# EryiXie/PlaneRecNet

Hardware: AMD Instinct MI355X
Metric: img/s fwd+bwd @480×640 ResNet101-DCN, 1/2/4/8 MI355X + roofline % (higher is better)
Workload: dtype f32 (tensors and accumulation fp32; plain GEMMs and the tap-walked 4x4/s2, 1x1/s2 and sub-pixel convolutions >= 300 tiles: 2xfp16-piece split MFMA, fp32 accumulate; fp32-only rate in fp32_only_run)

## Files before the change

### include/prn.h

```cpp
#ifndef PRN_H
#define PRN_H
#include <stdint.h>
#ifdef __cplusplus
extern "C" {
#endif

#define PRN_BN_SPLITS 32

int prn_version(void);
const char* prn_last_error(void);

enum { PRN_IN_ZERO = 0, PRN_IN_REFLECT = 1, PRN_IN_UP2_REFLECT = 2, PRN_IN_DILATED = 3, PRN_IN_UP2_PHASE = 4,
       PRN_IN_EMBED1 = 5  };
enum { PRN_EPI_NONE = 0, PRN_EPI_RELU = 1, PRN_EPI_SIGMOID = 2 };

enum { PRN_SPLIT_OFF = 0, PRN_SPLIT_PLAN = 1, PRN_SPLIT_ALWAYS = 2 };
enum { PRN_PIECES_BF16 = 0, PRN_PIECES_F16 = 16 };
typedef struct prn_gemm_opts {
  int32_t split_mode;
  int32_t split_kind;
  int32_t split_products;
  int32_t split_min_tiles;
  float split_min_gflop;
  int32_t wgrad_wgs;
// ... 65 lines not shown
int prn_winograd_input(const float* x, float* V, int B, int C, int H, int W, int in_mode, void* stream);
int64_t prn_gemm_batched_ws_bytes(int M, int C, int P, int nb, const prn_gemm_opts* opts);
int prn_gemm_batched(int M, int C, int P, int nb, const float* U, const void* u_images, const float* V, float* Y, void* ws, const prn_gemm_opts* opts,
                     void* stream);
int prn_winograd_output(const float* Y, const float* bias, const float* addend, float* y, int B, int M, int H, int W, int epilogue, void* stream);
int prn_winograd_output_bn_fwd(const float* Yt, float* x_out, float* stats, const float* gamma, const float* beta, float* y, float* running_mean,
                               float* running_var, int B, int M, int H, int W, float eps, float momentum, int relu, void* stream);
int prn_winograd_output_bn_bwd(const float* Yt, const float* x, const float* stats, const float* gamma, const float* beta, float* dx, float* dgamma,
                               float* dbeta, int B, int M, int H, int W, int relu, void* stream);
int64_t prn_winograd_wgrad_ws_bytes(int B, int C, int H, int W, int M, const prn_gemm_opts* opts);
int prn_winograd_dy(const float* dy, float* Y, int B, int M, int H, int W, void* stream);
int prn_gemm_batched_nt_splits(int M, int C, int P, int nb, const prn_gemm_opts* opts);
int prn_gemm_batched_nt_kind(int M, int C, int P, int nb, const prn_gemm_opts* opts);
int prn_gemm_batched_nt(int M, int C, int P, int nb, const float* A, const float* Bm, float* ws, const prn_gemm_opts* opts, void* stream);
int prn_winograd_dw(const float* partials, float* dw, int M, int C, int splits, void* stream);
int prn_conv3x3_winograd_wgrad(const float* x, const float* dy, float* dw, void* ws, int B, int C, int H, int W, int M, int in_mode, const prn_gemm_opts* opts,
                               void* stream, int phase);
int prn_conv3x3_winograd_wgrad_v(const float* V, const float* dy, float* dw, void* ws, int B, int C, int H, int W, int M, const prn_gemm_opts* opts, void* stream);
int64_t prn_winograd_tiles_ragged(const prn_ragged* rg, int B);
int64_t prn_conv3x3_winograd_ragged_ws_bytes(const prn_ragged* rg, int B, int C, int M, const prn_gemm_opts* opts);
int prn_conv3x3_winograd_ragged(const float* x, const float* U, const void* u_images, const float* bias, const float* addend, float* y, void* ws,
                                const prn_ragged* rg, int B, int C, int M, int epilogue, const prn_gemm_opts* opts, void* stream);
int64_t prn_winograd_wgrad_ragged_ws_bytes(const prn_ragged* rg, int B, int C, int M, const prn_gemm_opts* opts);
int prn_conv3x3_winograd_wgrad_ragged(const float* x, const float* dy, float* dw, void* ws, const prn_ragged* rg, int B, int C, int M, const prn_gemm_opts* opts,
                                      void* stream);
int64_t prn_conv3x3_winograd_ws_bytes(int B, int C, int H, int W, int M, const prn_gemm_opts* opts);
int prn_conv3x3_winograd(const float* x, const float* U, const void* u_images, const float* bias, const float* addend, float* y, void* ws, int B, int C, int H,
                         int W, int M, int in_mode, int epilogue, const prn_gemm_opts* opts, void* stream);

int64_t prn_conv2d_wgrad_ws_bytes(const prn_conv_desc* d);
int prn_conv2d_wgrad_kernel_kind(const prn_conv_desc* d, int G);
int prn_conv2d_wgrad(const prn_conv_desc* d, const float* x, const float* dy, float* dw, void* ws, void* stream);
#define PRN_WGRAD_GROUP_MAX 16
int64_t prn_conv2d_wgrad_grouped_ws_bytes(const prn_conv_desc* d, int G);
int prn_conv2d_wgrad_grouped(const prn_conv_desc* d, int G, const float* const* x, const float* const* dy, float* dw, void* ws, void* stream);
int prn_conv2d_wgrad_phase(const prn_conv_desc* d, const float* x, const float* dy, float* dw, void* ws, void* stream, int phase);

int prn_up2_phase_weights(const float* w, float* wp, int M, int C, void* stream);
int prn_up2_dgrad_weights(const float* w, float* kd, int M, int C, void* stream);
int prn_replicate_fold(const float* dp, float* dx, int B, int C, int H, int W, void* stream);
int prn_space_to_depth2(const float* in, float* out, int B, int C, int H, int W, void* stream);
int prn_up2_wgrad_combine(const float* dwp, float* dw, int M, int C, void* stream);

int prn_pad_fold(const float* dp, float* dx, int B, int C, int H, int W, int up2, void* stream);
int prn_pad_fold_pitched(const float* dp, float* dx, int B, int C, int H, int W, int pitch, void* stream);

int prn_channel_sum(const float* x, float* out, double* ws, int B, int C, int HW, void* stream);

int prn_dcn_sample(const float* x, const float* om, float* cols, int B, int C, int H, int W, int Ho, int Wo,
                   int stride, float max_offset, void* stream);
int64_t prn_dcn_sample_bwd_ws_bytes(int B, int C, int H, int W, int Ho, int Wo);
int prn_dcn_sample_bwd(const float* x, const float* om, const float* dcols, float* dx, float* d_om, void* ws,
                       int B, int C, int H, int W, int Ho, int Wo, int stride, float max_offset, void* stream);

typedef struct prn_dcn_desc {
  int32_t B, C, H, W;
  int32_t M;
  int32_t stride, pad;
  int32_t Ho, Wo;
  int32_t raw;
  float max_offset;
  int32_t epilogue;
  prn_gemm_opts opts;
} prn_dcn_desc;
int64_t prn_dcnv2_table_bytes(const prn_dcn_desc* d);
int prn_dcnv2_table(const prn_dcn_desc* d, const float* offset, const float* mask, void* table, void* stream);
int64_t prn_dcnv2_fwd_ws_bytes(const prn_dcn_desc* d);
int prn_dcnv2_fwd(const prn_dcn_desc* d, const float* x, const void* table, const float* w, const float* bias, float* y, void* ws, void* stream);
int prn_dcnv2_fwd_phase(const prn_dcn_desc* d, const float* x, const void* table, const float* w, const float* bias, float* y, void* ws, void* stream,
                        int phase);
int64_t prn_dcnv2_bwd_weight_ws_bytes(const prn_dcn_desc* d);
int prn_dcnv2_bwd_weight(const prn_dcn_desc* d, const float* x, const void* table, const float* dy, float* dw, void* ws, void* stream);
int prn_dcnv2_bwd_weight_phase(const prn_dcn_desc* d, const float* x, const void* table, const float* dy, float* dw, void* ws, void* stream, int phase);
int64_t prn_dcnv2_bwd_ws_bytes(const prn_dcn_desc* d);
int prn_dcnv2_bwd_input(const prn_dcn_desc* d, const float* dy, const float* wt, const void* wt_images, const float* offset, const float* mask, float* dx,
                        void* ws, void* stream);
int prn_dcnv2_bwd_input_phase(const prn_dcn_desc* d, const float* dy, const float* wt, const void* wt_images, const float* offset, const float* mask,
                              float* dx, void* ws, void* stream, int phase);
int prn_dcnv2_bwd_offset_mask(const prn_dcn_desc* d, const float* x, const float* offset, const float* mask, float* d_offset, float* d_mask,
                              void* ws, void* stream);

int prn_bn_stats(const float* x, float* stats, float* running_mean, float* running_var, double* ws,
                 int B, int C, int HW, float eps, float momentum, void* stream);
int prn_bn_apply(const float* x, const float* stats, const float* gamma, const float* beta, const float* residual,
                 float* y, int B, int C, int HW, int relu, void* stream);
int prn_bn_kernel_kind(int B, int HW);
int prn_bn_train_fwd(const float* x, float* stats, const float* gamma, const float* beta, const float* residual, float* y,
                     float* running_mean, float* running_var, double* ws, int B, int C, int HW, float eps, float momentum,
                     int relu, void* stream);
int prn_bn_bwd(const float* dy, const float* x, const float* y, const float* stats, const float* gamma, const float* beta,
               float* dx, float* dres, float* dgamma, float* dbeta, double* ws,
               int B, int C, int HW, int relu, int frozen, void* stream);
int prn_bn_train_fwd_into(const float* x, float* stats, const float* gamma, const float* beta, const float* residual, float* y,
                          int64_t y_batch_stride, float* running_mean, float* running_var, double* ws, int B, int C, int HW, float eps,
                          float momentum, int relu, void* stream);
int prn_bn_bwd_from(const float* dy, int64_t dy_batch_stride, const float* x, const float* y, const float* stats, const float* gamma,
                    const float* beta, float* dx, float* dres, float* dgamma, float* dbeta, double* ws,
                    int B, int C, int HW, int relu, int frozen, void* stream);

int prn_bn_train_fwd_partials(const float* parts, int nparts, int64_t part_stride, float* x_out, float* stats, const float* gamma, const float* beta,
                              const float* residual, float* y, float* running_mean, float* running_var, int B, int C, int HW, float eps, float momentum,
                              int relu, void* stream);
int prn_bn_bwd_partials(const float* dparts, int nparts, int64_t part_stride, const float* x, const float* y, const float* stats, const float* gamma,
                        const float* beta, float* dx, float* dres, float* dgamma, float* dbeta, int B, int C, int HW, int relu, int frozen, void* stream);
int prn_bn_train_fwd_winograd(const float* parts, int nparts, int64_t part_stride, float* x_out, float* stats, const float* gamma, const float* beta,
                              const float* residual, float* y, float* running_mean, float* running_var, float* V, int B, int C, int H, int W, float eps,
// ... 196 lines not shown
```

### planerecnet_amd/_lib.py

```python
import ctypes
import os

_HERE = os.path.dirname(os.path.abspath(__file__))
LIB_PATH = os.environ.get("PRN_LIB") or os.path.join(_HERE, "libprn_hip.so")

c_int, c_float, c_void_p, c_i64 = ctypes.c_int, ctypes.c_float, ctypes.c_void_p, ctypes.c_int64


class GemmOpts(ctypes.Structure):
    _fields_ = [("split_mode", ctypes.c_int32), ("split_kind", ctypes.c_int32), ("split_products", ctypes.c_int32), ("split_min_tiles", ctypes.c_int32),
                ("split_min_gflop", ctypes.c_float), ("wgrad_wgs", ctypes.c_int32), ("wgrad_target", ctypes.c_int32), ("wgrad_split", ctypes.c_int32)]

    def key(self):
        return (self.split_mode, self.split_kind, self.split_products, self.split_min_tiles, self.split_min_gflop, self.wgrad_wgs, self.wgrad_target, self.wgrad_split)


SPLIT_OFF, SPLIT_PLAN, SPLIT_ALWAYS = 0, 1, 2
PIECES_BF16, PIECES_F16 = 0, 16


class ConvDesc(ctypes.Structure):
    _fields_ = [(n, ctypes.c_int32) for n in
                ("B", "C", "H", "W", "M", "KH", "KW", "stride", "pad", "Ho", "Wo", "in_mode", "dil", "epilogue", "ystride", "yH", "yW", "reserved")] + [
                    ("opts", GemmOpts)]
# ... 38 lines not shown
    "prn_split_images_bytes": (c_i64, [c_int, c_int, c_int]),
    "prn_split_prepare": (c_int, [P, P, c_int, c_int, c_int, c_int, P]),
    "prn_split_prepare_batched": (c_int, [P, c_int, c_i64, c_i64, c_int, P]),
    "prn_conv2d_fwd": (c_int, [_DP, P, P, P, P, P, P, P]),
    "prn_conv2d_fwd_ragged": (c_int, [_DP, P, P, P, P, P, P, P]),
    "prn_conv2d_wgrad_ragged_ws_bytes": (c_i64, [_DP, P]),
    "prn_conv2d_wgrad_ragged": (c_int, [_DP, P, P, P, P, P, P]),
    "prn_gn_relu_fwd_ragged": (c_int, [P, P, P, P, P, c_int, c_int, c_int, P, c_int, c_float, P]),
    "prn_gn_relu_bwd_ragged": (c_int, [P, P, P, P, P, P, P, P, c_int, c_int, c_int, P, c_int, P]),
    "prn_conv2d_fwd_phase": (c_int, [_DP, P, P, P, P, P, P, P, c_int]),
    "prn_conv2d_fwd_counted": (c_int, [_DP, P, P, P, P, P, P, P, P, P, c_int]),
    "prn_conv2d_wgrad_phase": (c_int, [_DP, P, P, P, P, P, c_int]),
    "prn_weight_flip_transpose": (c_int, [P, P, c_int, c_int, c_int, c_int, P]),
    "prn_weight_flip_transpose_batched": (c_int, [P, c_int, c_i64, P]),
    "prn_winograd_tiles": (c_i64, [c_int, c_int, c_int]),
    "prn_winograd_weights_batched": (c_int, [P, c_int, c_i64, P]),
    "prn_winograd_input": (c_int, [P, P, c_int, c_int, c_int, c_int, c_int, P]),
    "prn_gemm_batched_ws_bytes": (c_i64, [c_int, c_int, c_int, c_int, _OP]),
    "prn_gemm_batched": (c_int, [c_int, c_int, c_int, c_int, P, P, P, P, P, _OP, P]),
    "prn_winograd_output": (c_int, [P, P, P, P, c_int, c_int, c_int, c_int, c_int, P]),
    "prn_winograd_output_bn_fwd": (c_int, [P] * 8 + [c_int] * 4 + [c_float, c_float, c_int, P]),
    "prn_winograd_output_bn_bwd": (c_int, [P] * 8 + [c_int] * 5 + [P]),
    "prn_winograd_wgrad_ws_bytes": (c_i64, [c_int] * 5 + [_OP]),
    "prn_winograd_dy": (c_int, [P, P, c_int, c_int, c_int, c_int, P]),
    "prn_gemm_batched_nt_splits": (c_int, [c_int] * 4 + [_OP]),
    "prn_gemm_batched_nt_kind": (c_int, [c_int] * 4 + [_OP]),
    "prn_conv2d_wgrad_kernel_kind": (c_int, [_DP, c_int]),
    "prn_gemm_batched_nt": (c_int, [c_int, c_int, c_int, c_int, P, P, P, _OP, P]),
    "prn_winograd_dw": (c_int, [P, P, c_int, c_int, c_int, P]),
    "prn_conv3x3_winograd_wgrad": (c_int, [P, P, P, P, c_int, c_int, c_int, c_int, c_int, c_int, _OP, P, c_int]),
    "prn_winograd_tiles_ragged": (c_i64, [P, c_int]),
    "prn_conv3x3_winograd_ragged_ws_bytes": (c_i64, [P, c_int, c_int, c_int, _OP]),
    "prn_conv3x3_winograd_ragged": (c_int, [P, P, P, P, P, P, P, P, c_int, c_int, c_int, c_int, _OP, P]),
    "prn_winograd_wgrad_ragged_ws_bytes": (c_i64, [P, c_int, c_int, c_int, _OP]),
    "prn_conv3x3_winograd_wgrad_ragged": (c_int, [P, P, P, P, P, c_int, c_int, c_int, _OP, P]),
    "prn_conv3x3_winograd_wgrad_v": (c_int, [P, P, P, P, c_int, c_int, c_int, c_int, c_int, _OP, P]),
    "prn_conv3x3_winograd_ws_bytes": (c_i64, [c_int] * 5 + [_OP]),
    "prn_conv3x3_winograd": (c_int, [P, P, P, P, P, P, P, c_int, c_int, c_int, c_int, c_int, c_int, c_int, _OP, P]),
    "prn_conv2d_wgrad_ws_bytes": (c_i64, [_DP]),
    "prn_conv2d_wgrad_grouped_ws_bytes": (c_i64, [_DP, c_int]),
    "prn_conv2d_wgrad_grouped": (c_int, [_DP, c_int, P, P, P, P, P]),
    "prn_conv2d_wgrad": (c_int, [_DP, P, P, P, P, P]),
    "prn_pad_fold": (c_int, [P, P, c_int, c_int, c_int, c_int, c_int, P]),
    "prn_pad_fold_pitched": (c_int, [P, P, c_int, c_int, c_int, c_int, c_int, P]),
    "prn_up2_phase_weights": (c_int, [P, P, c_int, c_int, P]),
    "prn_up2_dgrad_weights": (c_int, [P, P, c_int, c_int, P]),
    "prn_up2_wgrad_combine": (c_int, [P, P, c_int, c_int, P]),
    "prn_space_to_depth2": (c_int, [P, P, c_int, c_int, c_int, c_int, P]),
    "prn_replicate_fold": (c_int, [P, P, c_int, c_int, c_int, c_int, P]),
    "prn_channel_sum": (c_int, [P, P, P, c_int, c_int, c_int, P]),
    "prn_dcn_sample": (c_int, [P, P, P] + [c_int] * 7 + [c_float, P]),
    "prn_dcn_sample_bwd_ws_bytes": (c_i64, [c_int] * 6),
    "prn_dcn_sample_bwd": (c_int, [P, P, P, P, P, P] + [c_int] * 7 + [c_float, P]),
    "prn_dcnv2_table_bytes": (c_i64, [P]),
    "prn_dcnv2_table": (c_int, [P, P, P, P, P]),
    "prn_dcnv2_fwd_ws_bytes": (c_i64, [P]),
    "prn_dcnv2_fwd": (c_int, [P] * 8),
    "prn_dcnv2_fwd_phase": (c_int, [P] * 8 + [c_int]),
    "prn_dcnv2_bwd_weight_ws_bytes": (c_i64, [P]),
    "prn_dcnv2_bwd_weight": (c_int, [P] * 7),
    "prn_dcnv2_bwd_weight_phase": (c_int, [P] * 7 + [c_int]),
    "prn_dcnv2_bwd_ws_bytes": (c_i64, [P]),
    "prn_dcnv2_bwd_input": (c_int, [P] * 9),
    "prn_dcnv2_bwd_input_phase": (c_int, [P] * 9 + [c_int]),
    "prn_bn_kernel_kind": (c_int, [c_int, c_int]),
    "prn_dcnv2_bwd_offset_mask": (c_int, [P] * 8),
    "prn_plane_prior_ws_bytes": (c_i64, [c_int] * 6 + [_OP]),
    "prn_plane_prior_fwd": (c_int, [P] * 7 + [c_int] * 6 + [_OP, P]),
    "prn_plane_prior_fwd_phase": (c_int, [P] * 7 + [c_int] * 6 + [_OP, P, c_int]),
    "prn_plane_prior_wgrad_ws_bytes": (c_i64, [c_int] * 5 + [_OP]),
    "prn_plane_prior_wgrad": (c_int, [P] * 4 + [c_int] * 5 + [_OP, P]),
    "prn_fpn_level_ws_bytes": (c_i64, [c_int] * 8 + [_OP]),
    "prn_fpn_level_fwd": (c_int, [P, P, P, P, c_int, c_int, P, P, P, P, P, P] + [c_int] * 6 + [_OP, P]),
    "prn_frame_to_input": (c_int, [P] + [c_int] * 6 + [P, P, c_int, P, P, P]),
    "prn_mask_loss_ws_floats": (c_int, [c_int]),
    "prn_mask_loss_fwd": (c_int, [P] * 9 + [c_int, c_int, c_int, c_float, c_float, P]),
    "prn_mask_loss_bwd": (c_int, [P] * 8 + [c_int, c_int, P]),
    "prn_vnl_triplets": (c_int, [P] * 12 + [c_int, c_int, c_int, c_float, P]),
    "prn_vnl_scatter": (c_int, [P] * 5 + [c_int, c_int, P]),
    "prn_depth_metrics_ws_doubles": (c_int, []),
    "prn_depth_metrics": (c_int, [P, P, P, P, c_i64, c_float, c_float, P]),
    "prn_vnl_trim_key": (c_int, [P, P, P, P, c_int, P]),
    "prn_vnl_trim_fwd": (c_int, [P, P, P, P, P, P, P, c_int, c_int, c_int, P, P, P, P, P, P]),
    "prn_vnl_trim_ws_bytes": (c_i64, [c_int]),
    "prn_vnl_trim_bwd": (c_int, [P, P, P, P, P, P, P, c_int, c_int, P, P]),
    "prn_loss_ws_doubles": (c_int, [c_int]),
    "prn_focal_sum_fwd": (c_int, [P, P, P, P, c_i64, c_int, c_float, c_float, P]),
    "prn_focal_sum_bwd": (c_int, [P, P, P, P, c_i64, c_int, c_float, c_float, P]),
    "prn_rmse_log_fwd": (c_int, [P, P, P, P, P, c_int, c_int, c_float, c_float, P]),
    "prn_rmse_log_bwd": (c_int, [P, P, P, P, P, c_int, c_int, c_float, c_float, P]),
    "prn_gt_segments": (c_i64, [c_int, c_int]),
    "prn_gt_mask_stats": (c_int, [P, P, c_int, c_int, c_int, c_int, P, P, P, P]),
    "prn_gt_quarter_masks": (c_int, [P, P, c_int, c_int, c_int, P]),
    "prn_gt_sample_triplets": (c_int, [P, P, c_int, c_int, c_int, c_int, P, P, P, P, P, ctypes.c_uint64, ctypes.c_uint64, c_i64, P, P]),
    "prn_adam_chunk_elems": (c_int, []),
    "prn_adam_step": (c_int, [P, c_int, c_int, P, P, P, P, P, P, P, P, P, ctypes.c_double, ctypes.c_double, c_float, P]),
    "prn_adam_step_masked": (c_int, [P, c_int, c_int, P, P, P, P, P, P, P, P, P, ctypes.c_double, ctypes.c_double, c_float, P, P, P]),
    "prn_pairwise_iou_ws_bytes": (c_i64, [c_int, c_int, c_i64]),
    "prn_pairwise_iou": (c_int, [P, P, P, P, c_int, c_int, c_i64, P, P, P, P]),
    "prn_mask_boxes": (c_int, [P, c_int, c_int, c_int, P, P]),
    "prn_mask_stats": (c_int, [P, c_int, c_i64, c_float, P, P, P]),
    "prn_sigmoid_point_nms": (c_int, [P, P, c_int, c_int, c_int, c_i64, P]),
    "prn_matrix_nms": (c_int, [P, P, P, c_int, c_float, c_int, P, P, P]),
    "prn_mask_nms_ws_bytes": (c_i64, [c_int, c_int, c_i64]),
    "prn_mask_nms": (c_int, [P, P, P, P, c_int, c_int, c_i64, c_float, P, P, P]),
    "prn_bn_stats": (c_int, [P, P, P, P, P, c_int, c_int, c_int, c_float, c_float, P]),
# ... 71 lines not shown
```

### planerecnet_amd/csrc/prn_dcn.hip

```cpp
#include <stdlib.h>
#include "prn_common.h"

namespace {

struct Tap {
  int i00, i01, i10, i11;
  float w00, w01, w10, w11;
  float gy00, gy01, gy10, gy11, gx00, gx01, gx10, gx11;
  float mod;
  float sig;
  bool pass_y, pass_x;
};

struct OmView {
  const float* off; const float* msk;
  int64_t off_bs, msk_bs;
  float maxoff;
  int raw, pad;
};

__device__ __forceinline__ Tap make_tap(const OmView& v, int b, int k, int ho, int wo, int Ho, int Wo,
                                        int H, int W, int stride, bool need_grad) {
  Tap t;
  const size_t plane = (size_t)Ho * Wo, pix = (size_t)ho * Wo + wo;
  const float* ob = v.off + (size_t)b * v.off_bs;
  const float ry = ob[(2 * k) * plane + pix], rx = ob[(2 * k + 1) * plane + pix];
  float dy = ry, dx = rx;
  t.pass_y = t.pass_x = true;
  if (v.raw) {
    const float maxoff = v.maxoff;
    const float rm = ob[(18 + k) * plane + pix];
    dy = fminf(fmaxf(ry, -maxoff), maxoff); dx = fminf(fmaxf(rx, -maxoff), maxoff);
    t.pass_y = (ry >= -maxoff) && (ry <= maxoff);
    t.pass_x = (rx >= -maxoff) && (rx <= maxoff);
    t.sig = 1.f / (1.f + expf(-rm));
    t.mod = 2.f * t.sig;
  } else {
    t.sig = 0.f;
    t.mod = v.msk ? v.msk[(size_t)b * v.msk_bs + (size_t)k * plane + pix] : 1.f;
  }
  const int ki = k / 3, kj = k - ki * 3;
  const float y = (float)(ho * stride - v.pad + ki) + dy, x = (float)(wo * stride - v.pad + kj) + dx;
  const bool inside = (y > -1.f) && (y < (float)H) && (x > -1.f) && (x < (float)W);
  const float fy = floorf(y), fx = floorf(x);
  const int y0 = (int)fy, x0 = (int)fx, y1 = y0 + 1, x1 = x0 + 1;
  const float ly = y - fy, lx = x - fx, hy = 1.f - ly, hx = 1.f - lx;
  const bool vy0 = inside && y0 >= 0, vy1 = inside && y1 <= H - 1, vx0 = x0 >= 0, vx1 = x1 <= W - 1;
  const bool v00 = vy0 && vx0, v01 = vy0 && vx1, v10 = vy1 && vx0, v11 = vy1 && vx1;
  t.i00 = v00 ? y0 * W + x0 : 0; t.i01 = v01 ? y0 * W + x1 : 0;
  t.i10 = v10 ? y1 * W + x0 : 0; t.i11 = v11 ? y1 * W + x1 : 0;
  t.w00 = v00 ? hy * hx : 0.f; t.w01 = v01 ? hy * lx : 0.f;
  t.w10 = v10 ? ly * hx : 0.f; t.w11 = v11 ? ly * lx : 0.f;
  if (need_grad) {
    t.gy00 = v00 ? -hx : 0.f; t.gy01 = v01 ? -lx : 0.f; t.gy10 = v10 ? hx : 0.f; t.gy11 = v11 ? lx : 0.f;
    t.gx00 = v00 ? -hy : 0.f; t.gx01 = v01 ? hy : 0.f; t.gx10 = v10 ? -ly : 0.f; t.gx11 = v11 ? ly : 0.f;
  }
  return t;
}

__global__ __launch_bounds__(256) void dcn_sample_kernel(const float* __restrict__ x, OmView om,
                                                         float* __restrict__ cols, int B, int C, int H, int W, int Ho,
                                                         int Wo, int stride) {
  const int64_t gid = (int64_t)blockIdx.x * blockDim.x + threadIdx.x;
  const int64_t plane = (int64_t)Ho * Wo;
  if (gid >= (int64_t)B * 9 * plane) return;
  const int pix = gid % plane, k = (gid / plane) % 9, b = gid / (9 * plane);
  const int ho = pix / Wo, wo = pix - ho * Wo;
  const Tap t = make_tap(om, b, k, ho, wo, Ho, Wo, H, W, stride, false);
  const int cper = (C + gridDim.y - 1) / gridDim.y;
  const int c0 = blockIdx.y * cper, c1 = min(C, c0 + cper);
  const size_t HW = (size_t)H * W;
  const float* xp = x + ((size_t)b * C + c0) * HW;
  float* cp = cols + (((size_t)b * C + c0) * 9 + k) * plane + pix;
  constexpr int UN = 8;
  int c = c0;
  for (; c + UN <= c1; c += UN) {
    float a00[UN], a01[UN], a10[UN], a11[UN];
#pragma unroll
    for (int u = 0; u < UN; ++u) {
      const float* q = xp + (size_t)u * HW;
      a00[u] = q[t.i00]; a01[u] = q[t.i01]; a10[u] = q[t.i10]; a11[u] = q[t.i11];
    }
    __builtin_amdgcn_sched_barrier(0);
#pragma unroll
    for (int u = 0; u < UN; ++u) cp[(size_t)u * 9 * plane] = t.mod * (t.w00 * a00[u] + t.w01 * a01[u] + t.w10 * a10[u] + t.w11 * a11[u]);
    xp += (size_t)UN * HW;
    cp += (size_t)UN * 9 * plane;
  }
  for (; c < c1; ++c) {
    const float v = t.w00 * xp[t.i00] + t.w01 * xp[t.i01] + t.w10 * xp[t.i10] + t.w11 * xp[t.i11];
    *cp = t.mod * v;
    xp += HW;
    cp += 9 * plane;
  }
}

__global__ __launch_bounds__(256) void dcn_dom_partial_kernel(const float* __restrict__ x, OmView om,
                                                              const float* __restrict__ dcols, float* __restrict__ part, int B,
                                                              int C, int H, int W, int Ho, int Wo, int stride) {
  const int64_t gid = (int64_t)blockIdx.x * blockDim.x + threadIdx.x;
  const int64_t plane = (int64_t)Ho * Wo;
  if (gid >= (int64_t)B * 9 * plane) return;
  const int pix = gid % plane, k = (gid / plane) % 9, b = gid / (9 * plane);
  const int ho = pix / Wo, wo = pix - ho * Wo;
  const Tap t = make_tap(om, b, k, ho, wo, Ho, Wo, H, W, stride, true);
  const int cper = (C + gridDim.y - 1) / gridDim.y;
  const int c0 = blockIdx.y * cper, c1 = min(C, c0 + cper);
  const size_t HW = (size_t)H * W;
  const float* xp = x + ((size_t)b * C + c0) * HW;
  const float* dp = dcols + (((size_t)b * C + c0) * 9 + k) * plane + pix;
  float gy = 0.f, gx = 0.f, gm = 0.f;
  constexpr int UN = 8;
  int c = c0;
  for (; c + UN <= c1; c += UN) {
    float g[UN], a00[UN], a01[UN], a10[UN], a11[UN];
#pragma unroll
    for (int u = 0; u < UN; ++u) {
      const float* q = xp + (size_t)u * HW;
      g[u] = dp[(size_t)u * 9 * plane];
      a00[u] = q[t.i00]; a01[u] = q[t.i01]; a10[u] = q[t.i10]; a11[u] = q[t.i11];
    }
    __builtin_amdgcn_sched_barrier(0);
#pragma unroll
    for (int u = 0; u < UN; ++u) {
      gm += g[u] * (t.w00 * a00[u] + t.w01 * a01[u] + t.w10 * a10[u] + t.w11 * a11[u]);
      gy += g[u] * (t.gy00 * a00[u] + t.gy01 * a01[u] + t.gy10 * a10[u] + t.gy11 * a11[u]);
      gx += g[u] * (t.gx00 * a00[u] + t.gx01 * a01[u] + t.gx10 * a10[u] + t.gx11 * a11[u]);
    }
    xp += (size_t)UN * HW;
    dp += (size_t)UN * 9 * plane;
  }
  for (; c < c1; ++c) {
    const float g = *dp;
    const float x00 = xp[t.i00], x01 = xp[t.i01], x10 = xp[t.i10], x11 = xp[t.i11];
    gm += g * (t.w00 * x00 + t.w01 * x01 + t.w10 * x10 + t.w11 * x11);
    gy += g * (t.gy00 * x00 + t.gy01 * x01 + t.gy10 * x10 + t.gy11 * x11);
    gx += g * (t.gx00 * x00 + t.gx01 * x01 + t.gx10 * x10 + t.gx11 * x11);
    xp += HW;
    dp += 9 * plane;
  }
  float* ob = part + ((size_t)blockIdx.y * B + b) * 27 * plane + pix;
  ob[(2 * k) * plane] = t.pass_y ? gy * t.mod : 0.f;
  ob[(2 * k + 1) * plane] = t.pass_x ? gx * t.mod : 0.f;
  ob[(18 + k) * plane] = om.raw ? gm * 2.f * t.sig * (1.f - t.sig) : gm;
}

__global__ void dcn_dom_final_kernel(const float* __restrict__ part, float* __restrict__ d_off, float* __restrict__ d_msk, int64_t n, int G,
                                     int plane) {
  const int64_t i = (int64_t)blockIdx.x * blockDim.x + threadIdx.x;
  if (i >= n) return;
  float s = 0.f;
  for (int g = 0; g < G; ++g) s += part[(size_t)g * n + i];
  if (d_msk == nullptr) { d_off[i] = s; return; }
  const int64_t b = i / (27 * (int64_t)plane), r = i - b * 27 * (int64_t)plane;
  if (r < 18 * (int64_t)plane) d_off[b * 18 * plane + r] = s;
  else d_msk[b * 9 * plane + (r - 18 * (int64_t)plane)] = s;
}

struct CsrEntry { int src; float w; };

__device__ __forceinline__ bool csr_before(const CsrEntry& a, const CsrEntry& b) {
  return a.src < b.src || (a.src == b.src && __float_as_uint(a.w) < __float_as_uint(b.w));
}
__device__ __forceinline__ void csr_sort_bin(CsrEntry* __restrict__ e, int n) {
  if (n <= 8) {
    unsigned long long k[8];
    const unsigned long long* __restrict__ q = reinterpret_cast<const unsigned long long*>(e);
#pragma unroll
    for (int i = 0; i < 8; ++i) {
      const unsigned long long v = i < n ? q[i] : ~0ull;
      k[i] = i < n ? ((v << 32) | (v >> 32)) : ~0ull;
    }
#define PRN_CSR_CX(I, J) { const unsigned long long lo = k[I] < k[J] ? k[I] : k[J], hi = k[I] < k[J] ? k[J] : k[I]; k[I] = lo; k[J] = hi; }
    PRN_CSR_CX(0, 2) PRN_CSR_CX(1, 3) PRN_CSR_CX(4, 6) PRN_CSR_CX(5, 7) PRN_CSR_CX(0, 4) PRN_CSR_CX(1, 5) PRN_CSR_CX(2, 6) PRN_CSR_CX(3, 7)
    PRN_CSR_CX(0, 1) PRN_CSR_CX(2, 3) PRN_CSR_CX(4, 5) PRN_CSR_CX(6, 7) PRN_CSR_CX(2, 4) PRN_CSR_CX(3, 5) PRN_CSR_CX(1, 4) PRN_CSR_CX(3, 6)
    PRN_CSR_CX(1, 2) PRN_CSR_CX(3, 4) PRN_CSR_CX(5, 6)
#undef PRN_CSR_CX
    unsigned long long* __restrict__ o = reinterpret_cast<unsigned long long*>(e);
#pragma unroll
    for (int i = 0; i < 8; ++i)
      if (i < n) o[i] = (k[i] << 32) | (k[i] >> 32);
    return;
  }
  for (int i = 1; i < n; ++i) {
    const CsrEntry v = e[i];
    int j = i - 1;
    while (j >= 0 && csr_before(v, e[j])) { e[j + 1] = e[j]; --j; }
    e[j + 1] = v;
  }
}
__global__ __launch_bounds__(256) void dcn_csr_sort_kernel(const int* __restrict__ starts, const int* __restrict__ counts, CsrEntry* __restrict__ entries, int nbins) {
  const int bin = blockIdx.x * 256 + threadIdx.x;
  if (bin < nbins && counts[bin] > 1) csr_sort_bin(entries + starts[bin], counts[bin]);
}

__global__ __launch_bounds__(256) void dcn_csr_count_kernel(OmView om, int* __restrict__ counts, int B, int H, int W,
                                                            int Ho, int Wo, int stride) {
  const int64_t gid = (int64_t)blockIdx.x * blockDim.x + threadIdx.x;
  const int plane = Ho * Wo;
// ... 108 lines not shown
  for (int i = b0; i < b1; ++i) {
    const int c = csr_bins[i];
    starts[gb + i] = seg + off;
    counts[gb + i] = c;
    csr_bins[i] = off;
    off += c;
  }
  __syncthreads();
  for (int p = tid; p < plane; p += CSR1_THREADS) {
    const int ho = p / Wo, wo = p - ho * Wo;
    const Tap t = make_tap(om, b, k, ho, wo, Ho, Wo, H, W, stride, false);
    const int src = k * plane + p;
    if (t.w00 != 0.f) entries[seg + atomicAdd(csr_bins + t.i00, 1)] = CsrEntry{src, t.w00 * t.mod};
    if (t.w01 != 0.f) entries[seg + atomicAdd(csr_bins + t.i01, 1)] = CsrEntry{src, t.w01 * t.mod};
    if (t.w10 != 0.f) entries[seg + atomicAdd(csr_bins + t.i10, 1)] = CsrEntry{src, t.w10 * t.mod};
    if (t.w11 != 0.f) entries[seg + atomicAdd(csr_bins + t.i11, 1)] = CsrEntry{src, t.w11 * t.mod};
  }
  __syncthreads();
  for (int i = b0; i < b1; ++i) {
    const int beg = i > 0 ? csr_bins[i - 1] : 0, n = csr_bins[i] - beg;
    if (n > 1) csr_sort_bin(entries + seg + beg, n);
  }
}

template <int CH>
__global__ __launch_bounds__(256) void dcn_dx_gather_kernel(const float* __restrict__ dcols, const int* __restrict__ starts,
                                                            const int* __restrict__ counts, const CsrEntry* __restrict__ entries,
                                                            float* __restrict__ dx, int C, int HW, int plane) {
  const int q = blockIdx.x * 256 + threadIdx.x;
  if (q >= HW) return;
  const int b = blockIdx.z, c0 = blockIdx.y * CH;
  const size_t cstride = (size_t)9 * plane;
  const float* __restrict__ dp = dcols + ((size_t)b * C + c0) * cstride;
  float acc[CH];
#pragma unroll
  for (int cc = 0; cc < CH; ++cc) acc[cc] = 0.f;
  int st[9], cn[9];
#pragma unroll
  for (int k = 0; k < 9; ++k) {
    const size_t bin = (size_t)(b * 9 + k) * HW + q;
    st[k] = starts[bin];
    cn[k] = counts[bin];
  }
#pragma unroll
  for (int k = 0; k < 9; ++k) {
    const int s = st[k], n = cn[k];
    CsrEntry nxt;
    nxt.src = 0; nxt.w = 0.f;
    if (n > 0) nxt = entries[s];
    for (int e = s; e < s + n; ++e) {
      const CsrEntry en = nxt;
      if (e + 1 < s + n) nxt = entries[e + 1];
#pragma unroll
      for (int cc = 0; cc < CH; ++cc) acc[cc] += en.w * dp[cc * cstride + en.src];
    }
  }
  float* out = dx + ((size_t)b * C + c0) * HW + q;
#pragma unroll
  for (int cc = 0; cc < CH; ++cc)
    if (c0 + cc < C) out[(size_t)cc * HW] = acc[cc];
}

}

static int channel_groups(int C, int64_t threads) {
  static const int forced = prn_env_int("PRN_DCN_GROUPS", 0);
  int g = forced > 0 ? forced : (int)(1 + (256 * 8 * 256) / (threads > 0 ? threads : 1));
  if (g > 16) g = 16;
  if (g > C) g = C;
  while (g < C && C % g) ++g;
  return g < 1 ? 1 : g;
}

namespace {
OmView raw_view(const float* om, int Ho, int Wo, float max_offset) {
  OmView v;
  v.off = om; v.msk = nullptr; v.off_bs = v.msk_bs = (int64_t)27 * Ho * Wo; v.maxoff = max_offset; v.raw = 1; v.pad = 1;
  return v;
}
OmView desc_view(const prn_dcn_desc* d, const float* offset, const float* mask) {
  if (d->raw) { OmView v = raw_view(offset, d->Ho, d->Wo, d->max_offset); v.pad = d->pad; return v; }
  OmView v;
  v.off = offset; v.msk = mask; v.off_bs = (int64_t)18 * d->Ho * d->Wo; v.msk_bs = (int64_t)9 * d->Ho * d->Wo; v.maxoff = 0.f; v.raw = 0; v.pad = d->pad;
  return v;
}
}

extern "C" int prn_dcn_sample(const float* x, const float* om, float* cols, int B, int C, int H, int W, int Ho, int Wo,
                              int stride, float max_offset, void* stream) {
  PRN_REQUIRE(x && om && cols && B > 0 && C > 0 && H > 0 && W > 0 && Ho > 0 && Wo > 0, "prn_dcn_sample: bad arguments");
  PRN_REQUIRE(Ho == (H + 2 - 3) / stride + 1 && Wo == (W + 2 - 3) / stride + 1, "prn_dcn_sample: output size mismatch");
  const int64_t n = (int64_t)B * 9 * Ho * Wo;
  hipLaunchKernelGGL(dcn_sample_kernel, dim3(cdiv(n, 256), channel_groups(C, n)), dim3(256), 0, (hipStream_t)stream, x, raw_view(om, Ho, Wo, max_offset),
                     cols, B, C, H, W, Ho, Wo, stride);
  PRN_CHECK_LAUNCH("prn_dcn_sample");
  return 0;
}

namespace {
struct BwdWs { int64_t part, counts, starts, bsum, entries, total; int nbins, nblocks; };
BwdWs bwd_ws_layout(int B, int C, int H, int W, int Ho, int Wo) {
  auto up = [](int64_t v) { return (v + 255) / 256 * 256; };
  BwdWs l;
  l.nbins = B * 9 * H * W;
  l.nblocks = cdiv(l.nbins, SCAN_PER_BLOCK);
  l.part = 0;
  l.counts = up((int64_t)channel_groups(C, (int64_t)B * 9 * Ho * Wo) * B * 27 * Ho * Wo * 4);
  l.starts = l.counts + up((int64_t)l.nbins * 4);
  l.bsum = l.starts + up((int64_t)l.nbins * 4);
  l.entries = l.bsum + up((int64_t)l.nblocks * 4);
  l.total = l.entries + (int64_t)B * 9 * Ho * Wo * 4 * sizeof(CsrEntry);
  return l;
}

int launch_dom(const float* x, const OmView& v, const float* dcols, float* d_off, float* d_msk, char* wsb, const BwdWs& l, int B, int C, int H, int W,
               int Ho, int Wo, int stride, hipStream_t st) {
  const int64_t n = (int64_t)B * 9 * Ho * Wo;
  const int G = channel_groups(C, n);
  hipLaunchKernelGGL(dcn_dom_partial_kernel, dim3(cdiv(n, 256), G), dim3(256), 0, st, x, v, dcols, (float*)(wsb + l.part), B, C, H, W, Ho, Wo, stride);
  PRN_CHECK_LAUNCH("dcn d_om partial");
  const int64_t nom = (int64_t)B * 27 * Ho * Wo;
  hipLaunchKernelGGL(dcn_dom_final_kernel, dim3(cdiv(nom, 256)), dim3(256), 0, st, (const float*)(wsb + l.part), d_off, d_msk, nom, G, Ho * Wo);
  PRN_CHECK_LAUNCH("dcn d_om final");
  return 0;
}

int launch_dx(const OmView& v, const float* dcols, float* dx, char* wsb, const BwdWs& l, int B, int C, int H, int W, int Ho, int Wo, int stride,
              hipStream_t st) {
  const int64_t n = (int64_t)B * 9 * Ho * Wo;
  int* counts = (int*)(wsb + l.counts);
  int* starts = (int*)(wsb + l.starts);
  int* bsum = (int*)(wsb + l.bsum);
  CsrEntry* entries = (CsrEntry*)(wsb + l.entries);
  static const int one = prn_env_int("PRN_DCN_CSR1", 1);
  if (one && H * W <= CSR1_MAX_BINS) {
    hipLaunchKernelGGL(dcn_csr_build_kernel, dim3(B * 9), dim3(CSR1_THREADS), (size_t)H * W * sizeof(int), st, v, starts, counts, entries, H, W, Ho, Wo, stride);
  } else {
    if (hipMemsetAsync(counts, 0, (size_t)l.nbins * 4, st) != hipSuccess) { prn_set_error("dcn d-input: memset failed"); return 1; }
    hipLaunchKernelGGL(dcn_csr_count_kernel, dim3(cdiv(n, 256)), dim3(256), 0, st, v, counts, B, H, W, Ho, Wo, stride);
    hipLaunchKernelGGL(dcn_csr_block_sums_kernel, dim3(l.nblocks), dim3(256), 0, st, (const int*)counts, bsum, l.nbins);
    hipLaunchKernelGGL(dcn_csr_scan_kernel, dim3(l.nblocks), dim3(256), 0, st, counts, starts, (const int*)bsum, l.nbins);
    hipLaunchKernelGGL(dcn_csr_fill_kernel, dim3(cdiv(n, 256)), dim3(256), 0, st, v, (const int*)starts, counts, entries, B, H, W, Ho, Wo, stride);
    hipLaunchKernelGGL(dcn_csr_sort_kernel, dim3(cdiv(l.nbins, 256)), dim3(256), 0, st, (const int*)starts, (const int*)counts, entries, (int)l.nbins);
  }
  PRN_CHECK_LAUNCH("dcn d-input csr");
  const int HW = H * W;
  const int64_t blocks8 = (int64_t)cdiv(HW, 256) * cdiv(C, 8) * B;
  if (blocks8 >= 1024)
    hipLaunchKernelGGL((dcn_dx_gather_kernel<8>), dim3(cdiv(HW, 256), cdiv(C, 8), B), dim3(256), 0, st, dcols, (const int*)starts, (const int*)counts,
                       (const CsrEntry*)entries, dx, C, HW, Ho * Wo);
  else
    hipLaunchKernelGGL((dcn_dx_gather_kernel<4>), dim3(cdiv(HW, 256), cdiv(C, 4), B), dim3(256), 0, st, dcols, (const int*)starts, (const int*)counts,
                       (const CsrEntry*)entries, dx, C, HW, Ho * Wo);
  PRN_CHECK_LAUNCH("dcn d-input gather");
  return 0;
}
}

extern "C" int64_t prn_dcn_sample_bwd_ws_bytes(int B, int C, int H, int W, int Ho, int Wo) {
  if (B <= 0 || C <= 0 || H <= 0 || W <= 0 || Ho <= 0 || Wo <= 0 || (int64_t)B * 9 * H * W >= (1LL << 31)) return -1;
  return bwd_ws_layout(B, C, H, W, Ho, Wo).total;
}

extern "C" int prn_dcn_sample_bwd(const float* x, const float* om, const float* dcols, float* dx, float* d_om, void* ws,
                                  int B, int C, int H, int W, int Ho, int Wo, int stride, float max_offset, void* stream) {
  PRN_REQUIRE(x && om && dcols && dx && d_om && ws && B > 0 && C > 0, "prn_dcn_sample_bwd: bad arguments");
  PRN_REQUIRE((int64_t)B * 9 * H * W < (1LL << 31) && (int64_t)B * 36 * Ho * Wo < (1LL << 31), "prn_dcn_sample_bwd: map too large");
  hipStream_t st = (hipStream_t)stream;
  const BwdWs l = bwd_ws_layout(B, C, H, W, Ho, Wo);
  const OmView v = raw_view(om, Ho, Wo, max_offset);
  if (int e = launch_dom(x, v, dcols, d_om, nullptr, (char*)ws, l, B, C, H, W, Ho, Wo, stride, st)) return e;
  return launch_dx(v, dcols, dx, (char*)ws, l, B, C, H, W, Ho, Wo, stride, st);
// ... 68 lines not shown
```

Measured before the change: 191.5.

## Stage DCN offset-grad input window in LDS with double-buffered channel prefetch

Adds a new kernel for the DCN offset/mask gradient partials. Each block covers 64 pixels across all 9 taps and computes the span of bilinear sample indices the block touches. When that span fits the shared-memory budget, the block copies the window of x for 8 channels into LDS and gathers the four corners from there, fetching the next channels into registers while the current ones are used. Otherwise it falls back to direct global gathers unrolled by 8 and counts fallbacks in a workspace counter. The change adds block syncs and extra LDS use, and also fixes an out-of-range channel read in the CSR dx kernel.

```diff
diff --git a/include/prn.h b/include/prn.h
--- a/include/prn.h
+++ b/include/prn.h
@@ -141,6 +141,8 @@
 int64_t prn_dcn_sample_bwd_ws_bytes(int B, int C, int H, int W, int Ho, int Wo);
 int prn_dcn_sample_bwd(const float* x, const float* om, const float* dcols, float* dx, float* d_om, void* ws,
                        int B, int C, int H, int W, int Ho, int Wo, int stride, float max_offset, void* stream);
+int prn_dcn_bwd_staged(int mode);
+int prn_dcn_bwd_staged_budget(int window_floats);
 
 typedef struct prn_dcn_desc {
   int32_t B, C, H, W;
diff --git a/planerecnet_amd/_lib.py b/planerecnet_amd/_lib.py
--- a/planerecnet_amd/_lib.py
+++ b/planerecnet_amd/_lib.py
@@ -114,6 +114,8 @@
     "prn_dcn_sample": (c_int, [P, P, P] + [c_int] * 7 + [c_float, P]),
     "prn_dcn_sample_bwd_ws_bytes": (c_i64, [c_int] * 6),
     "prn_dcn_sample_bwd": (c_int, [P, P, P, P, P, P] + [c_int] * 7 + [c_float, P]),
+    "prn_dcn_bwd_staged": (c_int, [c_int]),
+    "prn_dcn_bwd_staged_budget": (c_int, [c_int]),
     "prn_dcnv2_table_bytes": (c_i64, [P]),
     "prn_dcnv2_table": (c_int, [P, P, P, P, P]),
     "prn_dcnv2_fwd_ws_bytes": (c_i64, [P]),
diff --git a/planerecnet_amd/csrc/prn_dcn.hip b/planerecnet_amd/csrc/prn_dcn.hip
--- a/planerecnet_amd/csrc/prn_dcn.hip
+++ b/planerecnet_amd/csrc/prn_dcn.hip
@@ -1,62 +1,11 @@
 #include <stdlib.h>
 #include "prn_common.h"
 
+#include "prn_dcn_geom.h"
+
 namespace {
 
-struct Tap {
-  int i00, i01, i10, i11;
-  float w00, w01, w10, w11;
-  float gy00, gy01, gy10, gy11, gx00, gx01, gx10, gx11;
-  float mod;
-  float sig;
-  bool pass_y, pass_x;
-};
-
-struct OmView {
-  const float* off; const float* msk;
-  int64_t off_bs, msk_bs;
-  float maxoff;
-  int raw, pad;
-};
-
-__device__ __forceinline__ Tap make_tap(const OmView& v, int b, int k, int ho, int wo, int Ho, int Wo,
-                                        int H, int W, int stride, bool need_grad) {
-  Tap t;
-  const size_t plane = (size_t)Ho * Wo, pix = (size_t)ho * Wo + wo;
-  const float* ob = v.off + (size_t)b * v.off_bs;
-  const float ry = ob[(2 * k) * plane + pix], rx = ob[(2 * k + 1) * plane + pix];
-  float dy = ry, dx = rx;
-  t.pass_y = t.pass_x = true;
-  if (v.raw) {
-    const float maxoff = v.maxoff;
-    const float rm = ob[(18 + k) * plane + pix];
-    dy = fminf(fmaxf(ry, -maxoff), maxoff); dx = fminf(fmaxf(rx, -maxoff), maxoff);
-    t.pass_y = (ry >= -maxoff) && (ry <= maxoff);
-    t.pass_x = (rx >= -maxoff) && (rx <= maxoff);
-    t.sig = 1.f / (1.f + expf(-rm));
-    t.mod = 2.f * t.sig;
-  } else {
-    t.sig = 0.f;
-    t.mod = v.msk ? v.msk[(size_t)b * v.msk_bs + (size_t)k * plane + pix] : 1.f;
-  }
-  const int ki = k / 3, kj = k - ki * 3;
-  const float y = (float)(ho * stride - v.pad + ki) + dy, x = (float)(wo * stride - v.pad + kj) + dx;
-  const bool inside = (y > -1.f) && (y < (float)H) && (x > -1.f) && (x < (float)W);
-  const float fy = floorf(y), fx = floorf(x);
-  const int y0 = (int)fy, x0 = (int)fx, y1 = y0 + 1, x1 = x0 + 1;
-  const float ly = y - fy, lx = x - fx, hy = 1.f - ly, hx = 1.f - lx;
-  const bool vy0 = inside && y0 >= 0, vy1 = inside && y1 <= H - 1, vx0 = x0 >= 0, vx1 = x1 <= W - 1;
-  const bool v00 = vy0 && vx0, v01 = vy0 && vx1, v10 = vy1 && vx0, v11 = vy1 && vx1;
-  t.i00 = v00 ? y0 * W + x0 : 0; t.i01 = v01 ? y0 * W + x1 : 0;
-  t.i10 = v10 ? y1 * W + x0 : 0; t.i11 = v11 ? y1 * W + x1 : 0;
-  t.w00 = v00 ? hy * hx : 0.f; t.w01 = v01 ? hy * lx : 0.f;
-  t.w10 = v10 ? ly * hx : 0.f; t.w11 = v11 ? ly * lx : 0.f;
-  if (need_grad) {
-    t.gy00 = v00 ? -hx : 0.f; t.gy01 = v01 ? -lx : 0.f; t.gy10 = v10 ? hx : 0.f; t.gy11 = v11 ? lx : 0.f;
-    t.gx00 = v00 ? -hy : 0.f; t.gx01 = v01 ? hy : 0.f; t.gx10 = v10 ? -ly : 0.f; t.gx11 = v11 ? ly : 0.f;
-  }
-  return t;
-}
+using namespace prn_dcn_geom;
 
 __global__ __launch_bounds__(256) void dcn_sample_kernel(const float* __restrict__ x, OmView om,
                                                          float* __restrict__ cols, int B, int C, int H, int W, int Ho,
@@ -93,6 +42,32 @@
     xp += HW;
     cp += 9 * plane;
   }
+}
+
+template <bool FIRST00>
+__device__ __forceinline__ float dom_dot(float w00, float w01, float w10, float w11, float a00, float a01, float a10, float a11) {
+  const float s = FIRST00 ? __builtin_fmaf(w01, a01, w00 * a00) : __builtin_fmaf(w00, a00, w01 * a01);
+  return __builtin_fmaf(w11, a11, __builtin_fmaf(w10, a10, s));
+}
+template <bool FIRST00_Y>
+__device__ __forceinline__ void dom_acc_1(const Tap& t, float g, float x00, float x01, float x10, float x11, float& gm, float& gy, float& gx) {
+  gm = __builtin_fmaf(g, dom_dot<false>(t.w00, t.w01, t.w10, t.w11, x00, x01, x10, x11), gm);
+  gy = __builtin_fmaf(g, dom_dot<FIRST00_Y>(t.gy00, t.gy01, t.gy10, t.gy11, x00, x01, x10, x11), gy);
+  gx = __builtin_fmaf(g, dom_dot<false>(t.gx00, t.gx01, t.gx10, t.gx11, x00, x01, x10, x11), gx);
+}
+template <int N>
+__device__ __forceinline__ void dom_acc_un(const Tap& t, const float (&g)[N], const float (&a00)[N], const float (&a01)[N], const float (&a10)[N],
+                                           const float (&a11)[N], float& gm, float& gy, float& gx) {
+#pragma unroll
+  for (int u = 0; u < N; ++u) {
+    if ((u & 3) == 3) dom_acc_1<true>(t, g[u], a00[u], a01[u], a10[u], a11[u], gm, gy, gx);
+    else dom_acc_1<false>(t, g[u], a00[u], a01[u], a10[u], a11[u], gm, gy, gx);
+  }
+}
+__device__ __forceinline__ void dom_store(const Tap& t, int raw, float* __restrict__ ob, int k, size_t plane, float gm, float gy, float gx) {
+  ob[(2 * k) * plane] = t.pass_y ? gy * t.mod : 0.f;
+  ob[(2 * k + 1) * plane] = t.pass_x ? gx * t.mod : 0.f;
+  ob[(18 + k) * plane] = raw ? gm * 2.f * t.sig * (1.f - t.sig) : gm;
 }
 
 __global__ __launch_bounds__(256) void dcn_dom_partial_kernel(const float* __restrict__ x, OmView om,
@@ -145,6 +120,130 @@
   ob[(18 + k) * plane] = om.raw ? gm * 2.f * t.sig * (1.f - t.sig) : gm;
 }
 
+template <bool VEC>
+__device__ __forceinline__ float4 dom_load4(const float* __restrict__ g, int r) {
+  if (VEC) return *reinterpret_cast<const float4*>(g);
+  float4 v;
+  v.x = g[0];
+  v.y = r > 1 ? g[1] : 0.f;
+  v.z = r > 2 ? g[2] : 0.f;
+  v.w = r > 3 ? g[3] : 0.f;
+  return v;
+}
+
+template <bool VEC>
+__global__ __launch_bounds__(DOM_THREADS, 5) void dcn_dom_staged_kernel(const float* __restrict__ x, OmView om, const float* __restrict__ dcols,
+                                                                     float* __restrict__ part, int B, int C, int H, int W, int Ho, int Wo, int stride,
+                                                                     int budget, unsigned* __restrict__ stats) {
+  __shared__ __attribute__((aligned(16))) float win[DOM_UN * DOM_WIN_MAX];
+  __shared__ int red[18];
+  const int tid = threadIdx.x, k = tid >> 6, lane = tid & 63;
+  const int b = blockIdx.z, plane = Ho * Wo;
+  const int p = blockIdx.x * DOM_TILE + lane;
+  const bool live = p < plane;
+  const int pix = live ? p : plane - 1;
+  const int ho = pix / Wo, wo = pix - ho * Wo;
+  const Tap t = make_tap(om, b, k, ho, wo, Ho, Wo, H, W, stride, true);
+  int lo, hi;
+  tap_span(t, lo, hi);
+#pragma unroll
+  for (int o = 32; o > 0; o >>= 1) { lo = min(lo, __shfl_xor(lo, o)); hi = max(hi, __shfl_xor(hi, o)); }
+  if (lane == 0) { red[k] = lo; red[9 + k] = hi; }
+  __syncthreads();
+#pragma unroll
+  for (int i = 0; i < 9; ++i) { lo = min(lo, red[i]); hi = max(hi, red[9 + i]); }
+  const DomWindow w = dom_window(lo, hi, budget);
+  const int cper = (C + gridDim.y - 1) / gridDim.y;
+  const int c0 = blockIdx.y * cper, c1 = min(C, c0 + cper);
+  const size_t HW = (size_t)H * W;
+  const float* dp = dcols + (((size_t)b * C + c0) * 9 + k) * plane + pix;
+  float gy = 0.f, gx = 0.f, gm = 0.f;
+  if (!w.staged) {
+    if (tid == 0) atomicAdd(stats, 1u);
+    const float* xp = x + ((size_t)b * C + c0) * HW;
+    int c = c0;
+    for (; c + DOM_UN <= c1; c += DOM_UN) {
+#pragma unroll
+      for (int h = 0; h < 2; ++h) {
+        float g[4], a00[4], a01[4], a10[4], a11[4];
+#pragma unroll
+        for (int u = 0; u < 4; ++u) {
+          const float* q = xp + (size_t)u * HW;
+          g[u] = dp[(size_t)u * 9 * plane];
+          a00[u] = q[t.i00]; a01[u] = q[t.i01]; a10[u] = q[t.i10]; a11[u] = q[t.i11];
+        }
+        dom_acc_un<4>(t, g, a00, a01, a10, a11, gm, gy, gx);
+        xp += (size_t)4 * HW;
+        dp += (size_t)4 * 9 * plane;
+      }
+    }
+    for (; c < c1; ++c) {
+      dom_acc_1<false>(t, *dp, xp[t.i00], xp[t.i01], xp[t.i10], xp[t.i11], gm, gy, gx);
+      xp += HW;
+      dp += 9 * (size_t)plane;
+    }
+  } else {
+    const int s00 = dom_slot(w, t.i00, t.vmask & 1u), s01 = dom_slot(w, t.i01, t.vmask & 2u);
+    const int s10 = dom_slot(w, t.i10, t.vmask & 4u), s11 = dom_slot(w, t.i11, t.vmask & 8u);
+    const float* xb = x + (size_t)b * C * HW;
+    static_assert(DOM_VEC_PER_THREAD == 4, "the staging registers below are written out");
+    constexpr int SF = DOM_THREADS / DOM_UN;
+    const int su = tid / SF, sf = tid - su * SF;
+    const float* sq = xb + (size_t)(c0 + su) * HW + w.base + 4 * sf;
+    float* sl = win + su * DOM_WIN_MAX + 4 * sf;
+    const int rem = (int)HW - w.base - 4 * sf;
+    const bool m0 = sf < w.nvec, m1 = sf + SF < w.nvec, m2 = sf + 2 * SF < w.nvec, m3 = sf + 3 * SF < w.nvec;
+    float4 g0, g1, g2, g3;
+    g0 = g1 = g2 = g3 = make_float4(0.f, 0.f, 0.f, 0.f);
+#define PRN_DOM_FETCH(nch_)                                                    \
+    if (su < (nch_)) {                                                         \
+      if (m0) g0 = dom_load4<VEC>(sq, rem);                                    \
+      if (m1) g1 = dom_load4<VEC>(sq + 4 * SF, rem - 4 * SF);                  \
+      if (m2) g2 = dom_load4<VEC>(sq + 8 * SF, rem - 8 * SF);                  \
+      if (m3) g3 = dom_load4<VEC>(sq + 12 * SF, rem - 12 * SF);                \
+    }
+#define PRN_DOM_PUT(nch_)                                                      \
+    if (su < (nch_)) {                                                         \
+      if (m0) *reinterpret_cast<float4*>(sl) = g0;                             \
+      if (m1) *reinterpret_cast<float4*>(sl + 4 * SF) = g1;                    \
+      if (m2) *reinterpret_cast<float4*>(sl + 8 * SF) = g2;                    \
+      if (m3) *reinterpret_cast<float4*>(sl + 12 * SF) = g3;                   \
+    }
+    int c = c0, nch = min(DOM_UN, c1 - c0);
+    if (c < c1) { PRN_DOM_FETCH(nch) }
+    while (c < c1) {
+      __syncthreads();
+      PRN_DOM_PUT(nch)
+      __syncthreads();
+      const int cn = c + nch, nn = min(DOM_UN, c1 - cn);
+      if (nch == DOM_UN) {
+        float g[DOM_UN], a00[DOM_UN], a01[DOM_UN], a10[DOM_UN], a11[DOM_UN];
+#pragma unroll
+        for (int u = 0; u < DOM_UN; ++u) g[u] = dp[(size_t)u * 9 * plane];
+        sq += (size_t)DOM_UN * HW;
+        if (cn < c1) { PRN_DOM_FETCH(nn) }
+#pragma unroll
+        for (int u = 0; u < DOM_UN; ++u) {
+          const float* q = win + u * DOM_WIN_MAX;
+          a00[u] = q[s00]; a01[u] = q[s01]; a10[u] = q[s10]; a11[u] = q[s11];
+        }
+        dom_acc_un<DOM_UN>(t, g, a00, a01, a10, a11, gm, gy, gx);
+        dp += (size_t)DOM_UN * 9 * plane;
+      } else {
+        for (int u = 0; u < nch; ++u) {
+          const float* q = win + u * DOM_WIN_MAX;
+          dom_acc_1<false>(t, *dp, q[s00], q[s01], q[s10], q[s11], gm, gy, gx);
+          dp += 9 * (size_t)plane;
+        }
+      }
+      c = cn; nch = nn;
+    }
+  }
+#undef PRN_DOM_FETCH
+#undef PRN_DOM_PUT
+  if (live) dom_store(t, om.raw, part + ((size_t)blockIdx.y * B + b) * 27 * plane + pix, k, (size_t)plane, gm, gy, gx);
+}
+
 __global__ void dcn_dom_final_kernel(const float* __restrict__ part, float* __restrict__ d_off, float* __restrict__ d_msk, int64_t n, int G,
                                      int plane) {
   const int64_t i = (int64_t)blockIdx.x * blockDim.x + threadIdx.x;
@@ -359,7 +458,7 @@
       const CsrEntry en = nxt;
       if (e + 1 < s + n) nxt = entries[e + 1];
 #pragma unroll
-      for (int cc = 0; cc < CH; ++cc) acc[cc] += en.w * dp[cc * cstride + en.src];
+      for (int cc = 0; cc < CH; ++cc) acc[cc] += en.w * dp[(c0 + cc < C ? cc : 0) * cstride + en.src];
     }
   }
   float* out = dx + ((size_t)b * C + c0) * HW + q;
@@ -368,6 +467,24 @@
     if (c0 + cc < C) out[(size_t)cc * HW] = acc[cc];
 }
 
+}
+
+static int dcn_staged_mode = -1, dcn_dom_budget = DOM_WIN_MAX;
+static int dcn_staged() {
+  if (dcn_staged_mode < 0) {
+    static const int env = prn_env_int("PRN_DCN_BWD_STAGED", 1);
+    dcn_staged_mode = env != 0;
+  }
+  return dcn_staged_mode;
+}
+extern "C" int prn_dcn_bwd_staged(int mode) {
+  const int was = dcn_staged();
+  if (mode >= 0) dcn_staged_mode = mode != 0;
+  return was;
+}
+extern "C" int prn_dcn_bwd_staged_budget(int window_floats) {
+  dcn_dom_budget = window_floats > 0 && window_floats < DOM_WIN_MAX ? window_floats : DOM_WIN_MAX;
+  return 0;
 }
 
 static int channel_groups(int C, int64_t threads) {
@@ -405,7 +522,7 @@
 }
 
 namespace {
-struct BwdWs { int64_t part, counts, starts, bsum, entries, total; int nbins, nblocks; };
+struct BwdWs { int64_t part, counts, starts, bsum, entries, stats, total; int nbins, nblocks; };
 BwdWs bwd_ws_layout(int B, int C, int H, int W, int Ho, int Wo) {
   auto up = [](int64_t v) { return (v + 255) / 256 * 256; };
   BwdWs l;
@@ -416,7 +533,8 @@
   l.starts = l.counts + up((int64_t)l.nbins * 4);
   l.bsum = l.starts + up((int64_t)l.nbins * 4);
   l.entries = l.bsum + up((int64_t)l.nblocks * 4);
-  l.total = l.entries + (int64_t)B * 9 * Ho * Wo * 4 * sizeof(CsrEntry);
+  l.stats = l.entries + up((int64_t)B * 9 * Ho * Wo * 4 * sizeof(CsrEntry));
+  l.total = l.stats + 256;
   return l;
 }
 
@@ -424,7 +542,12 @@
                int Ho, int Wo, int stride, hipStream_t st) {
   const int64_t n = (int64_t)B * 9 * Ho * Wo;
   const int G = channel_groups(C, n);
-  hipLaunchKernelGGL(dcn_dom_partial_kernel, dim3(cdiv(n, 256), G), dim3(256), 0, st, x, v, dcols, (float*)(wsb + l.part), B, C, H, W, Ho, Wo, stride);
+  const bool vec = (((size_t)H * W) & 3) == 0 && ((uintptr_t)x & 15) == 0;
+  if (dcn_staged() && B <= 65535)
+    hipLaunchKernelGGL(vec ? dcn_dom_staged_kernel<true> : dcn_dom_staged_kernel<false>, dim3(cdiv((int64_t)Ho * Wo, DOM_TILE), G, B), dim3(DOM_THREADS), 0, st, x, v, dcols, (float*)(wsb + l.part), B, C, H, W,
+                       Ho, Wo, stride, dcn_dom_budget, (unsigned*)(wsb + l.stats));
+  else
+    hipLaunchKernelGGL(dcn_dom_partial_kernel, dim3(cdiv(n, 256), G), dim3(256), 0, st, x, v, dcols, (float*)(wsb + l.part), B, C, H, W, Ho, Wo, stride);
   PRN_CHECK_LAUNCH("dcn d_om partial");
   const int64_t nom = (int64_t)B * 27 * Ho * Wo;
   hipLaunchKernelGGL(dcn_dom_final_kernel, dim3(cdiv(nom, 256)), dim3(256), 0, st, (const float*)(wsb + l.part), d_off, d_msk, nom, G, Ho * Wo);
diff --git a/planerecnet_amd/csrc/prn_dcn_geom.h b/planerecnet_amd/csrc/prn_dcn_geom.h
--- /dev/null
+++ b/planerecnet_amd/csrc/prn_dcn_geom.h
@@ -0,0 +1,101 @@
+#pragma once
+#include <math.h>
+#include <stddef.h>
+#include <stdint.h>
+
+#if defined(__HIPCC__)
+#define PRN_HD __host__ __device__ __forceinline__
+#else
+#define PRN_HD inline
+#endif
+
+namespace prn_dcn_geom {
+
+struct Tap {
+  int i00, i01, i10, i11;
+  float w00, w01, w10, w11;
+  float gy00, gy01, gy10, gy11, gx00, gx01, gx10, gx11;
+  float mod;
+  float sig;
+  bool pass_y, pass_x;
+  unsigned vmask;
+};
+
+struct OmView {
+  const float* off; const float* msk;
+  int64_t off_bs, msk_bs;
+  float maxoff;
+  int raw, pad;
+};
+
+PRN_HD Tap make_tap(const OmView& v, int b, int k, int ho, int wo, int Ho, int Wo, int H, int W, int stride, bool need_grad) {
+  Tap t;
+  const size_t plane = (size_t)Ho * Wo, pix = (size_t)ho * Wo + wo;
+  const float* ob = v.off + (size_t)b * v.off_bs;
+  const float ry = ob[(2 * k) * plane + pix], rx = ob[(2 * k + 1) * plane + pix];
+  float dy = ry, dx = rx;
+  t.pass_y = t.pass_x = true;
+  if (v.raw) {
+    const float maxoff = v.maxoff;
+    const float rm = ob[(18 + k) * plane + pix];
+    dy = fminf(fmaxf(ry, -maxoff), maxoff); dx = fminf(fmaxf(rx, -maxoff), maxoff);
+    t.pass_y = (ry >= -maxoff) && (ry <= maxoff);
+    t.pass_x = (rx >= -maxoff) && (rx <= maxoff);
+    t.sig = 1.f / (1.f + expf(-rm));
+    t.mod = 2.f * t.sig;
+  } else {
+    t.sig = 0.f;
+    t.mod = v.msk ? v.msk[(size_t)b * v.msk_bs + (size_t)k * plane + pix] : 1.f;
+  }
+  const int ki = k / 3, kj = k - ki * 3;
+  const float y = (float)(ho * stride - v.pad + ki) + dy, x = (float)(wo * stride - v.pad + kj) + dx;
+  const bool inside = (y > -1.f) && (y < (float)H) && (x > -1.f) && (x < (float)W);
+  const float fy = floorf(y), fx = floorf(x);
+  const int y0 = (int)fy, x0 = (int)fx, y1 = y0 + 1, x1 = x0 + 1;
+  const float ly = y - fy, lx = x - fx, hy = 1.f - ly, hx = 1.f - lx;
+  const bool vy0 = inside && y0 >= 0, vy1 = inside && y1 <= H - 1, vx0 = x0 >= 0, vx1 = x1 <= W - 1;
+  const bool v00 = vy0 && vx0, v01 = vy0 && vx1, v10 = vy1 && vx0, v11 = vy1 && vx1;
+  t.i00 = v00 ? y0 * W + x0 : 0; t.i01 = v01 ? y0 * W + x1 : 0;
+  t.i10 = v10 ? y1 * W + x0 : 0; t.i11 = v11 ? y1 * W + x1 : 0;
+  t.w00 = v00 ? hy * hx : 0.f; t.w01 = v01 ? hy * lx : 0.f;
+  t.w10 = v10 ? ly * hx : 0.f; t.w11 = v11 ? ly * lx : 0.f;
+  t.vmask = (v00 ? 1u : 0u) | (v01 ? 2u : 0u) | (v10 ? 4u : 0u) | (v11 ? 8u : 0u);
+  if (need_grad) {
+    t.gy00 = v00 ? -hx : 0.f; t.gy01 = v01 ? -lx : 0.f; t.gy10 = v10 ? hx : 0.f; t.gy11 = v11 ? lx : 0.f;
+    t.gx00 = v00 ? -hy : 0.f; t.gx01 = v01 ? hy : 0.f; t.gx10 = v10 ? -ly : 0.f; t.gx11 = v11 ? ly : 0.f;
+  }
+  return t;
+}
+
+constexpr int DOM_TILE = 64;
+constexpr int DOM_THREADS = 9 * DOM_TILE;
+constexpr int DOM_UN = 8;
+constexpr int DOM_VEC_PER_THREAD = 4;
+constexpr int DOM_WIN_MAX = DOM_VEC_PER_THREAD * DOM_THREADS / DOM_UN * 4;
+
+PRN_HD void tap_span(const Tap& t, int& lo, int& hi) {
+  lo = 0x7fffffff; hi = -1;
+  if (t.vmask & 1u) { lo = t.i00 < lo ? t.i00 : lo; hi = t.i00 > hi ? t.i00 : hi; }
+  if (t.vmask & 2u) { lo = t.i01 < lo ? t.i01 : lo; hi = t.i01 > hi ? t.i01 : hi; }
+  if (t.vmask & 4u) { lo = t.i10 < lo ? t.i10 : lo; hi = t.i10 > hi ? t.i10 : hi; }
+  if (t.vmask & 8u) { lo = t.i11 < lo ? t.i11 : lo; hi = t.i11 > hi ? t.i11 : hi; }
+}
+
+struct DomWindow {
+  int base;
+  int nvec;
+  int pitch;
+  bool staged;
+};
+PRN_HD DomWindow dom_window(int lo, int hi, int budget) {
+  DomWindow w;
+  if (hi < lo) { lo = 0; hi = 0; }
+  w.base = lo & ~3;
+  w.nvec = (hi - w.base) / 4 + 1;
+  w.pitch = 4 * w.nvec;
+  w.staged = w.pitch <= budget;
+  return w;
+}
+PRN_HD int dom_slot(const DomWindow& w, int idx, bool valid) { return valid ? idx - w.base : 0; }
+
+}
```

Result: no change. 192.2, median of 6 (+0.4%).
